# isl-org/adaptive-surface-reconstruction

Measured on AMD Instinct MI355X. Metric: input points/sec to signed implicit values, higher is better.
Workload: dtype f32 via bf16x3 (24-bit operands, f32 accumulate)

## Files before the change

### adaptive-surface-reconstruction_amd/csrc/asr_api.hip

```cpp
#include <cmath>
#include <cstdlib>
#include <cstring>

#include <algorithm>
#include <functional>
#include <future>
#include <mutex>
#include <thread>

#include "asr_common.h"
#include "asr_uset.h"

#define ASR_ROW_GROUP_SEGMENT (ctx->opt.row_segment > 0 ? ctx->opt.row_segment : (i64)524288)
#define CTX_GUARD(ctx)                                                  \
    if (!(ctx)) return ASR_HIP_EINVAL;                                  \
    (ctx)->err.clear();                                                 \
    if (hipSetDevice((ctx)->device) != hipSuccess) {                    \
        (ctx)->err = "hipSetDevice failed for the context's device";   \
        return ASR_HIP_EHIP;                                            \
    }

namespace {
struct OptEntry {
    const char* name;
    const char* env;
    i64 AsrOptions::*field;
};
const OptEntry k_options[] = {
        {"sconv_min_blocks", "ASR_SCONV_MIN_BLOCKS", &AsrOptions::sconv_min_blocks},
        {"sconv_wide_min", "ASR_SCONV_WIDE_MIN", &AsrOptions::sconv_wide_min},
        {"row_segment", "ASR_ROW_SEGMENT", &AsrOptions::row_segment},
        {"row_lpt", "ASR_ROW_LPT", &AsrOptions::row_lpt},
        {"row_ranked", "ASR_ROW_RANKED", &AsrOptions::row_ranked},
        {"sconv_plan", "ASR_SCONV_PLAN", &AsrOptions::sconv_plan},
        {"plan_arena", "ASR_PLAN_ARENA", &AsrOptions::plan_arena},
        {"sconv16_min_blocks", "ASR_SCONV16_MIN_BLOCKS", &AsrOptions::sconv16_min_blocks},
        {"knn_cells", "ASR_KNN_CELLS", &AsrOptions::knn_cells},
        {"knn_deep", "ASR_KNN_DEEP", &AsrOptions::knn_deep},
        {"search_hash_level", "ASR_SEARCH_HASH_LEVEL", &AsrOptions::search_hash_level},
        {"overlap", "ASR_OVERLAP", &AsrOptions::overlap},
        {"build_search", "ASR_BUILD_SEARCH", &AsrOptions::build_search},
        {"cconv_valu", "ASR_CCONV_VALU", &AsrOptions::cconv_valu},
        {"search_half", "ASR_SEARCH_HALF", &AsrOptions::search_half},
        {"search_priority", "ASR_SEARCH_PRIORITY", &AsrOptions::search_priority},
        {"shard_timing", "ASR_SHARD_TIMING", &AsrOptions::shard_timing},
        {"shard_geometry", "ASR_SHARD_GEOMETRY", &AsrOptions::shard_geometry},
        {"early_sort", "ASR_EARLY_SORT", &AsrOptions::early_sort},
        {"early_cells", "ASR_EARLY_CELLS", &AsrOptions::early_cells},
        {"sconv_split_rows", "ASR_SCONV_SPLIT_ROWS", &AsrOptions::sconv_split_rows},
        {"sconv_split_min_rows", "ASR_SCONV_SPLIT_MIN_ROWS", &AsrOptions::sconv_split_min_rows},
        {"arena_cap_mb", "ASR_ARENA_CAP_MB", &AsrOptions::arena_cap_mb},
        {"inject_failure", "ASR_INJECT_FAILURE", &AsrOptions::inject_failure},
};
void apply_arena_cap(asr_hip_context* ctx) {
    const size_t cap = ctx->opt.arena_cap_mb > 0 ? (size_t)ctx->opt.arena_cap_mb << 20 : 0;
    for (asr_hip_context* c : {ctx, ctx->aux})
        if (c) c->persist.cap = c->scratch.cap = c->shard_mem.cap = cap;
}

struct PrintSlot {
    asr_hip_print_callback cb = nullptr;
    void* user = nullptr;
};
std::mutex g_print_mu;
PrintSlot g_print[4];
}

extern "C" {

const char* asr_hip_version(void) { return "0.2.0+mi355x.r6"; }

int asr_hip_set_print_callback(asr_hip_print_callback callback, void* user, const int* levels, int num_levels) {
    if (num_levels < 0 || (num_levels > 0 && !levels)) return ASR_HIP_EINVAL;
    for (int i = 0; i < num_levels; ++i)
        if (levels[i] < ASR_HIP_DEBUG || levels[i] > ASR_HIP_ERROR) return ASR_HIP_EINVAL;
    std::lock_guard<std::mutex> lock(g_print_mu);
    for (int i = 0; i < num_levels; ++i) g_print[levels[i]] = PrintSlot{callback, callback ? user : nullptr};
    return ASR_HIP_OK;
}
void asr_hip_print(const char* msg, int level) {
    if (!msg || level < ASR_HIP_DEBUG || level > ASR_HIP_ERROR) return;
    PrintSlot s;
    {
        std::lock_guard<std::mutex> lock(g_print_mu);
        s = g_print[level];
    }
    if (s.cb) s.cb(msg, s.user);
}

size_t asr_hip_struct_size(const char* name) {
    if (!name) return 0;
    if (!strcmp(name, "asr_octree_frame")) return sizeof(asr_octree_frame);
    if (!strcmp(name, "asr_sparse_conv_args")) return sizeof(asr_sparse_conv_args);
    if (!strcmp(name, "asr_weight")) return sizeof(asr_weight);
    if (!strcmp(name, "asr_implicit_params")) return sizeof(asr_implicit_params);
    if (!strcmp(name, "asr_implicit_sizes")) return sizeof(asr_implicit_sizes);
    if (!strcmp(name, "asr_shard_comm")) return sizeof(asr_shard_comm);
    if (!strcmp(name, "asr_shard_stats")) return sizeof(asr_shard_stats);
    if (!strcmp(name, "asr_mesh_topology")) return sizeof(asr_mesh_topology);
    return 0;
}

int asr_hip_context_create(asr_hip_context** out, void* stream) {
    if (!out) return ASR_HIP_EINVAL;
    *out = nullptr;
    int ndev = 0;
    if (hipGetDeviceCount(&ndev) != hipSuccess || ndev <= 0) return ASR_HIP_ENODEV;
    asr_hip_context* ctx = new asr_hip_context();
    ctx->stream = (hipStream_t)stream;
    (void)hipGetDevice(&ctx->device);
    memset(&ctx->sizes, 0, sizeof(ctx->sizes));
    for (const OptEntry& o : k_options)
        if (const char* e = getenv(o.env)) ctx->opt.*(o.field) = atoll(e);
    apply_arena_cap(ctx);
    *out = ctx;
    return ASR_HIP_OK;
// ... 1661 lines not shown
```

### adaptive-surface-reconstruction_amd/csrc/asr_common.h

```cpp
#pragma once
#include <hip/hip_runtime.h>

#include <cstdint>
#include <cstdio>
#include <map>
#include <string>
#include <tuple>
#include <vector>

#include "../../include/asr_hip.h"

typedef uint64_t u64;
typedef int64_t i64;
typedef uint32_t u32;

struct Arena {
    struct Slab {
        char* base;
        size_t size, used;
    };
    std::vector<Slab> slabs;
    size_t min_slab = size_t(256) << 20;
    size_t cap = 0;

    void* alloc(size_t bytes) {
        bytes = (bytes + 255) & ~size_t(255);
        if (bytes == 0) bytes = 256;
        for (auto& s : slabs)
            if (s.size - s.used >= bytes) {
                void* p = s.base + s.used;
                s.used += bytes;
                return p;
            }
        size_t sz = bytes > min_slab ? bytes : min_slab;
        if (cap && reserved() + sz > cap) return nullptr;
        void* p = nullptr;
        if (hipMalloc(&p, sz) != hipSuccess) return nullptr;
        slabs.push_back({(char*)p, sz, bytes});
        return p;
    }
    void reset() {
        for (auto& s : slabs) s.used = 0;
    }
    size_t reserved() const {
        size_t t = 0;
        for (auto& s : slabs) t += s.size;
        return t;
    }
    void release() {
        for (auto& s : slabs) (void)hipFree(s.base);
        slabs.clear();
    }
};

struct ArenaMark {
    std::vector<size_t> used;
};
static inline void arena_mark(const Arena& a, ArenaMark& m) {
    m.used.clear();
    for (auto& s : a.slabs) m.used.push_back(s.used);
}
static inline void arena_rewind(Arena& a, const ArenaMark& m) {
    for (size_t i = 0; i < a.slabs.size(); ++i) a.slabs[i].used = i < m.used.size() ? m.used[i] : 0;
}

struct GridDev {
    i64 v = 0, p = 0;
    u64* keys = nullptr;
    float* centers = nullptr;
    float* sizes = nullptr;
    int32_t* nidx = nullptr;
    uint8_t* nkidx = nullptr;
    i64* nrs = nullptr;
    int32_t* up_idx = nullptr;
    uint8_t* up_kidx = nullptr;
    i64* up_rs = nullptr;
    int32_t* down_idx = nullptr;
    uint8_t* down_kidx = nullptr;
    i64* down_rs = nullptr;
    int32_t* perm_nb = nullptr;
    int32_t* perm_up = nullptr;
    int32_t* perm_down = nullptr;
};

struct AsrOptions {
    i64 sconv_min_blocks = 2816;
    i64 sconv16_min_blocks = 1024;
    i64 sconv_wide_min = 2048;
    i64 row_segment = 524288;
    i64 search_hash_level = -1;
    i64 knn_deep = 1;
    i64 knn_cells = 1;
    i64 plan_arena = 0;
    i64 sconv_plan = 1;
    i64 row_ranked = 1;
    i64 row_lpt = 1;
    i64 overlap = 1;
    i64 cconv_valu = 0;
    i64 build_search = 1;
    i64 shard_geometry = -1;
    i64 shard_timing = 0;
    i64 search_priority = 2;
    i64 search_half = 1;
    i64 early_cells = 1;
    i64 early_sort = 1;
    i64 arena_cap_mb = 0;
    i64 inject_failure = 0;
    i64 sconv_split_min_rows = 2048;
    i64 sconv_split_rows = 32768;
};

struct asr_conv_plan_view {
    const uint4* hdr;
    const int32_t* pool;
    i64 groups;
    unsigned pool_bytes;
};
struct asr_conv_plan {
    uint4* hdr = nullptr;
    int32_t* pool = nullptr;
    i64 groups = 0, groups_pad = 0, blocks = 0;
    i64* offs = nullptr;
    const int32_t* nidx = nullptr;
    const uint8_t* kidx = nullptr;
    const i64* rs = nullptr;
    const int32_t* perm = nullptr;
    i64 num_out = 0;
    int K = 0;
    bool usable() const { return hdr && blocks * 64 < (i64(1) << 32) - 65536; }
    asr_conv_plan_view view() const { return {hdr, pool, groups, (unsigned)(blocks * 64)}; }
};

struct AsrPointIndex {
    bool valid = false;
    const float* pts = nullptr;
    const float* radii = nullptr;
    i64 n = 0;
    int lsort = 0;
    float4* sorted = nullptr;
    int32_t* ids = nullptr;
    int32_t* rank = nullptr;
    float* srad = nullptr;
    u64* codes = nullptr;
    u64* tab_keys = nullptr;
    u64 tab_mask = 0;
    int32_t* tab_start = nullptr;
    int32_t* tab_end = nullptr;
    int tab_lmin = 0, tab_lmax = -1, tab_lhash = 0, tab_grow = 0;
};

struct asr_hip_context {
    hipStream_t stream = nullptr;
    std::string err;
    AsrOptions opt;
    std::map<const void*, asr_conv_plan> conv_plans;
    std::map<std::string, i64> sconv_launches;
    ArenaMark build_mark;
    bool build_mark_ok = false;
    Arena persist;
    Arena scratch;
    Arena plan_arena;
    uint64_t plan_arena_epoch = 0;
    u64* nodes = nullptr;
    u64* leaves = nullptr;
    i64 num_nodes = 0, num_leaves = 0;
    asr_octree_frame frame;
    asr_implicit_sizes sizes;
    GridDev grids[ASR_NUM_GRIDS];
    int32_t* agg_idx = nullptr;
    float* agg_dist = nullptr;
    float* agg_compat = nullptr;
    i64* agg_rs = nullptr;
    int32_t* agg_spos = nullptr;
    const float4* agg_sorted = nullptr;
    bool has_search = false;
    bool build_sharded = false;
    const int32_t* agg_rows = nullptr;
    i64 agg_nq = 0;
    const float* agg_qcenters = nullptr;
// ... 306 lines not shown
```

### adaptive-surface-reconstruction_amd/csrc/asr_geom.hip

```cpp
#include <cstdlib>
#include <cstring>
#include <algorithm>
#include <rocprim/rocprim.hpp>

#include "asr_common.h"
#include "asr_prim.h"

namespace {
using namespace asr_prim;

constexpr int BLK = 256;

struct HashTab {
    u64* keys;
    int32_t* vals;
    u64 mask;
};

struct TabProbe {
    u64 bucket, step, low, bmask;
    __device__ inline u64 slot() const { return ((bucket & bmask) << 6) | low; }
    __device__ inline void next() { bucket += step; }
};
__device__ inline TabProbe tab_probe(const HashTab& t, u64 key) {
    const u64 h = asr_hash64(key >> 6);
    return TabProbe{h, (h >> 32) | 1, key & 63, t.mask >> 6};
}

__device__ inline u64 ld_agent(const u64* p) {
    return __hip_atomic_load(p, __ATOMIC_RELAXED, __HIP_MEMORY_SCOPE_AGENT);
}

__device__ inline int tab_insert(const HashTab& t, u64 key, u64* slot_out = nullptr) {
    TabProbe pr = tab_probe(t, key);
    for (u64 probe = 0; probe <= pr.bmask; ++probe, pr.next()) {
        const u64 slot = pr.slot();
        u64 cur = ld_agent(&t.keys[slot]);
        if (cur == 0) {
            cur = atomicCAS((unsigned long long*)&t.keys[slot], 0ull, (unsigned long long)key);
            if (cur == 0) {
                if (slot_out) *slot_out = slot;
                return 1;
            }
        }
        if (cur == key) {
            if (slot_out) *slot_out = slot;
            return 0;
        }
    }
    return -1;
}
__device__ inline int tab_insert_shared(const HashTab& t, u64 key) {
    TabProbe pr = tab_probe(t, key);
    for (u64 probe = 0; probe <= pr.bmask; ++probe, pr.next()) {
        const u64 slot = pr.slot();
        u64 cur = t.keys[slot];
        if (cur == 0) cur = ld_agent(&t.keys[slot]);
        if (cur == 0) {
            cur = atomicCAS((unsigned long long*)&t.keys[slot], 0ull, (unsigned long long)key);
            if (cur == 0) return 1;
        }
        if (cur == key) return 0;
    }
    return -1;
}
__device__ inline bool tab_contains(const HashTab& t, u64 key) {
    TabProbe pr = tab_probe(t, key);
    for (u64 probe = 0; probe <= pr.bmask; ++probe, pr.next()) {
        const u64 slot = pr.slot();
        const u64 cur = t.keys[slot];
        if (cur == key) return true;
        if (cur == 0) return false;
    }
    return false;
}
__device__ inline int tab_find(const HashTab& t, u64 key) {
    TabProbe pr = tab_probe(t, key);
    for (u64 probe = 0; probe <= pr.bmask; ++probe, pr.next()) {
        const u64 slot = pr.slot();
        const u64 cur = t.keys[slot];
        if (cur == key) return t.vals[slot];
        if (cur == 0) return -1;
    }
    return -1;
}
__device__ inline i64 tab_find_slot(const HashTab& t, u64 key) {
    TabProbe pr = tab_probe(t, key);
    for (u64 probe = 0; probe <= pr.bmask; ++probe, pr.next()) {
        const u64 slot = pr.slot();
// ... 1770 lines not shown
    const int j = rg_job_of(b, c * 128);
    const i64 r0 = c * 128 - b.base[j];
    u64 m0 = masks[sorted_ids[c * 128 + lane]], m1 = masks[sorted_ids[c * 128 + 64 + lane]];
#pragma unroll
    for (int o = 32; o > 0; o >>= 1) {
        m0 |= __shfl_xor(m0, o, 64);
        m1 |= __shfl_xor(m1, o, 64);
    }
    if (lane == 0) {
        int cost = __popcll(m0) + __popcll(m1);
        if (r0 + 128 > b.v[j]) cost = 0;
        ckey[c] = (int32_t)(((i64)j << 13) | ((r0 / seg) << 7) | (127 - cost));
        cid[c] = (int32_t)c;
    }
}
__global__ void k_rg_apply(RowGroupBatch b, const int32_t* sorted_ids, const int32_t* order, int lpt) {
    const i64 e = blockIdx.x * (i64)blockDim.x + threadIdx.x;
    if (e >= b.base[b.n]) return;
    const int j = rg_job_of(b, e);
    const i64 r = e - b.base[j];
    if (r >= b.v[j]) return;
    const i64 src = lpt ? (i64)order[e >> 7] * 128 + (e & 127) : e;
    b.out[j][r] = (int32_t)(sorted_ids[src] - b.base[j]);
}

constexpr int RG_MAX_MASKS = 16384;
constexpr int RG_MASK_TAB = 65536;
__global__ void k_rg_masks(RowGroupBatch b, u64* masks, HashTab t, int* cnt) {
    const i64 e = blockIdx.x * (i64)blockDim.x + threadIdx.x;
    if (e >= b.base[b.n]) return;
    const int j = rg_job_of(b, e);
    const i64 r = e - b.base[j];
    u64 m = 0;
    if (r < b.v[j]) {
        const i64* rs = b.rs[j];
        const uint8_t* kidx = b.kidx[j];
        for (i64 p = rs[r]; p < rs[r + 1]; ++p) m |= u64(1) << (kidx[p] & 63);
        if (tab_insert_shared(t, (m >> 1) + 1) < 0) cnt[1] = 1;
    }
    masks[e] = m;
}
__global__ void k_rg_mask_collect(HashTab t, u64* list, int32_t* slot_of, int* cnt) {
    const u64 i = blockIdx.x * (u64)blockDim.x + threadIdx.x;
    const u64 k = i <= t.mask ? t.keys[i] : 0;
    const int o = block_append(k != 0, cnt + 2);
    if (k && o < RG_MAX_MASKS) {
        list[o] = k;
        slot_of[o] = (int32_t)i;
    }
}
__global__ __launch_bounds__(256) void k_rg_mask_ranks(HashTab t, const u64* list, const int32_t* slot_of, const int* cnt) {
    __shared__ u64 s_key[2048];
    const int n = cnt[2];
    if (n > RG_MAX_MASKS) return;
    const int i = blockIdx.x * blockDim.x + threadIdx.x;
    if (blockIdx.x * blockDim.x >= n) return;
    const u64 mine = i < n ? list[i] : 0;
    int rank = 0;
    for (int base = 0; base < n; base += 2048) {
        __syncthreads();
        for (int e = threadIdx.x; e < 2048; e += blockDim.x) s_key[e] = base + e < n ? list[base + e] : ~u64(0);
        __syncthreads();
        const int m = min(2048, n - base);
        for (int e = 0; e < m; ++e) rank += s_key[e] < mine;
    }
    if (i < n) t.vals[slot_of[i]] = rank;
}
__global__ void k_rg_keys_ranked(RowGroupBatch b, i64 seg, const u64* masks, HashTab t, unsigned* keys, int32_t* ids,
                                 int rank_bits) {
    const i64 e = blockIdx.x * (i64)blockDim.x + threadIdx.x;
    if (e >= b.base[b.n]) return;
    const int j = rg_job_of(b, e);
    const i64 r = e - b.base[j];
    unsigned key;
    if (r < b.v[j]) {
        const int rank = tab_find(t, (masks[e] >> 1) + 1);
        key = ((unsigned)j << (6 + rank_bits)) | ((unsigned)(r / seg) << rank_bits) | (unsigned)rank;
    } else {
        key = ((unsigned)j << (6 + rank_bits)) | (63u << rank_bits) | ((1u << rank_bits) - 1u);
    }
    keys[e] = key;
    ids[e] = (int32_t)e;
}

__device__ inline u64 dev_morton_add(u64 a, u64 b) {
    const u64 M = 0x9249249249249249ull;
    u64 c = ((a | ~M) + (b & M)) & M;
    c |= ((a | ~(M << 1)) + (b & (M << 1))) & (M << 1);
    c |= ((a | ~(M << 2)) + (b & (M << 2))) & (M << 2);
    return c;
}
__device__ inline u64 dev_morton_sub(u64 a, u64 b) {
    const u64 M = 0x9249249249249249ull;
    u64 c = ((a & M) - (b & M)) & M;
    c |= ((a & (M << 1)) - (b & (M << 1))) & (M << 1);
    c |= ((a & (M << 2)) - (b & (M << 2))) & (M << 2);
    return c;
}
__device__ inline int node_lookup(const HashTab& t, u64 key) {
    TabProbe pr = tab_probe(t, key);
    for (u64 probe = 0; probe <= pr.bmask; ++probe, pr.next()) {
        const u64 slot = pr.slot();
        const u64 cur = t.keys[slot];
        if (cur == key) return t.vals[slot];
        if (cur == 0) return -2;
    }
    return -2;
}
__device__ inline bool dual_owned(const HashTab& t, u64 key, int i, u64& vertex_key) {
    const u64 IM = 0x9249249249249249ull;
    const int lev = asr_key_level(key);
    const u64 min_lev_key = u64(1) << (3 * lev);
    const u64 vk = dev_morton_add(key, (u64)i);
    const u64 vk_ = vk - min_lev_key;
    if (vk >= (min_lev_key << 1) || !(vk_ & IM) || !(vk_ & (IM << 1)) || !(vk_ & (IM << 2))) return false;
    vertex_key = vk;
    for (int j = 0; j < 8; ++j) {
        if (j == i) continue;
        const u64 ak = dev_morton_sub(vk, (u64)j);
        const int r = node_lookup(t, ak);
        if (r == -2) continue;
        if (r == -1) return false;
        if (ak < key) return false;
    }
    return true;
}
__global__ void k_dual_count(const u64* leaves, i64 v, HashTab t, i64* counts) {
    i64 q = blockIdx.x * (i64)blockDim.x + threadIdx.x;
    if (q > v) return;
    if (q == v) {
        counts[v] = 0;
        return;
    }
    const u64 key = leaves[q];
    int n = 0;
    u64 vk;
    for (int i = 0; i < 8; ++i) n += dual_owned(t, key, i, vk) ? 1 : 0;
    counts[q] = n;
}
__global__ void k_dual_fill(const u64* leaves, i64 v, HashTab t, const i64* offsets, i64* out, int* cnt) {
    i64 q = blockIdx.x * (i64)blockDim.x + threadIdx.x;
    if (q >= v) return;
    const u64 key = leaves[q];
    i64 o = offsets[q];
    for (int i = 0; i < 8; ++i) {
        u64 vk;
        if (!dual_owned(t, key, i, vk)) continue;
        for (int j = 0; j < 8; ++j) {
            u64 k = dev_morton_sub(vk, (u64)j);
            int r = -2;
            while (k != 0 && (r = node_lookup(t, k)) == -2) k >>= 3;
            if (k == 0 || r < 0) {
                cnt[1] = 1;
                r = -1;
            }
            out[o * 8 + j] = r;
        }
        ++o;
    }
}

int make_table(asr_hip_context* ctx, Arena& arena, u64 cap, bool with_vals, HashTab& t) {
    t.keys = arena_alloc<u64>(arena, cap);
    t.vals = with_vals ? arena_alloc<int32_t>(arena, cap) : nullptr;
    t.mask = cap - 1;
    if (!t.keys || (with_vals && !t.vals)) ASR_FAIL(ctx, ASR_HIP_EHIP, "arena allocation failed");
// ... 364 lines not shown
        ASR_CHECK_LAUNCH(ctx);
        k_chunk_key<<<grid_for(nc, BLK), BLK, 0, ctx->stream>>>(tcost, v, seg, ckey, cid);
        ASR_CHECK_LAUNCH(ctx);
        ASR_TRY((sort_pairs<int32_t, int32_t>(ctx, ctx->scratch, ckey, ckey_s, cid, cid_s, nc,
                                              7 + bits_for((v + seg - 1) / seg + 1))));
        k_chunk_apply<<<grid_for(v, BLK), BLK, 0, ctx->stream>>>(perm_m, cid_s, v, perm_out);
        ASR_CHECK_LAUNCH(ctx);
    }
    return ASR_HIP_OK;
}

static int rg_batch_run(asr_hip_context* ctx, const asr_row_group_job* jobs, int n, i64 seg, int mask_bits);
static int rg_batch_run_ranked(asr_hip_context* ctx, const asr_row_group_job* jobs, int n, i64 seg, bool* done);
int asr_geom_row_groups_batch(asr_hip_context* ctx, const asr_row_group_job* jobs, int n, i64 seg) {
    if (seg < 128) seg = 128;
    bool fits = n <= RG_MAX_JOBS && seg % 128 == 0;
    for (int j = 0; j < n && fits; ++j) fits = jobs[j].v / seg < 63 && jobs[j].v < (i64(1) << 31);
    if (!fits) {
        for (int j = 0; j < n; ++j)
            ASR_TRY(asr_geom_row_groups(ctx, jobs[j].kidx, jobs[j].rs, jobs[j].v, seg, jobs[j].perm_out, jobs[j].kbits));
        return ASR_HIP_OK;
    }
    if (ctx->opt.row_ranked) {
        bool done = false;
        ASR_TRY(rg_batch_run_ranked(ctx, jobs, n, seg, &done));
        if (done) return ASR_HIP_OK;
    }
    std::vector<asr_row_group_job> small_jobs, wide_jobs;
    for (int j = 0; j < n; ++j) (jobs[j].kbits <= 10 ? small_jobs : wide_jobs).push_back(jobs[j]);
    if (!small_jobs.empty()) ASR_TRY(rg_batch_run(ctx, small_jobs.data(), (int)small_jobs.size(), seg, 9));
    if (!wide_jobs.empty()) ASR_TRY(rg_batch_run(ctx, wide_jobs.data(), (int)wide_jobs.size(), seg, 54));
    return ASR_HIP_OK;
}
static int rg_batch_run_ranked(asr_hip_context* ctx, const asr_row_group_job* jobs, int n, i64 seg, bool* done) {
    *done = false;
    ASR_TRY(ensure_flags(ctx));
    RowGroupBatch b;
    b.n = 0;
    i64 total = 0;
    for (int j = 0; j < n; ++j) {
        if (jobs[j].v <= 0) continue;
        b.base[b.n] = total;
        b.v[b.n] = jobs[j].v;
        b.kidx[b.n] = jobs[j].kidx;
        b.rs[b.n] = jobs[j].rs;
        b.out[b.n] = jobs[j].perm_out;
        total += (jobs[j].v + 127) / 128 * 128;
        ++b.n;
    }
    if (b.n == 0) {
        *done = true;
        return ASR_HIP_OK;
    }
    b.base[b.n] = total;
    if (total >= (i64(1) << 31)) ASR_FAIL(ctx, ASR_HIP_EINVAL, "row_groups: too many rows");
    u64* masks = arena_alloc<u64>(ctx->scratch, total);
    unsigned* keys = arena_alloc<unsigned>(ctx->scratch, total);
    unsigned* keys_s = arena_alloc<unsigned>(ctx->scratch, total);
    int32_t* ids = arena_alloc<int32_t>(ctx->scratch, total);
    int32_t* ids_s = arena_alloc<int32_t>(ctx->scratch, total);
    const i64 nc = total / 128;
    int32_t* ckey = arena_alloc<int32_t>(ctx->scratch, nc);
    int32_t* ckey_s = arena_alloc<int32_t>(ctx->scratch, nc);
    int32_t* cid = arena_alloc<int32_t>(ctx->scratch, nc);
    int32_t* cid_s = arena_alloc<int32_t>(ctx->scratch, nc);
    if (!masks || !keys || !keys_s || !ids || !ids_s || !ckey || !ckey_s || !cid || !cid_s)
        ASR_FAIL(ctx, ASR_HIP_EHIP, "arena allocation failed");
    HashTab t;
    ASR_TRY(make_table(ctx, ctx->scratch, RG_MASK_TAB, true, t));
    ASR_TRY(fresh_flags(ctx));
    k_rg_masks<<<grid_for(total, BLK), BLK, 0, ctx->stream>>>(b, masks, t, ctx->d_flags);
    ASR_CHECK_LAUNCH(ctx);
    u64* mlist = arena_alloc<u64>(ctx->scratch, RG_MAX_MASKS);
    int32_t* mslot = arena_alloc<int32_t>(ctx->scratch, RG_MAX_MASKS);
    if (!mlist || !mslot) ASR_FAIL(ctx, ASR_HIP_EHIP, "arena allocation failed");
    k_rg_mask_collect<<<grid_for((i64)t.mask + 1, BLK), BLK, 0, ctx->stream>>>(t, mlist, mslot, ctx->d_flags);
    ASR_CHECK_LAUNCH(ctx);
    k_rg_mask_ranks<<<RG_MAX_MASKS / 256, 256, 0, ctx->stream>>>(t, mlist, mslot, ctx->d_flags);
    ASR_CHECK_LAUNCH(ctx);
    int host[16];
    ASR_TRY(read_flags(ctx, host));
    if (host[1] || host[2] > RG_MAX_MASKS) return ASR_HIP_OK;
    const int rank_bits = bits_for(std::max(host[2], 2));
    k_rg_keys_ranked<<<grid_for(total, BLK), BLK, 0, ctx->stream>>>(b, seg, masks, t, keys, ids, rank_bits);
    ASR_CHECK_LAUNCH(ctx);
    ASR_TRY((sort_pairs<unsigned, int32_t>(ctx, ctx->scratch, keys, keys_s, ids, ids_s, total, 4 + 6 + rank_bits)));
    const int lpt = ctx->opt.row_lpt != 0;
    if (lpt) {
        k_rg_chunk_keys<<<grid_for(nc * 64, BLK), BLK, 0, ctx->stream>>>(b, seg, ids_s, masks, ckey, cid);
        ASR_CHECK_LAUNCH(ctx);
        ASR_TRY((sort_pairs<int32_t, int32_t>(ctx, ctx->scratch, ckey, ckey_s, cid, cid_s, nc, 17)));
    }
    k_rg_apply<<<grid_for(total, BLK), BLK, 0, ctx->stream>>>(b, ids_s, cid_s, lpt);
    ASR_CHECK_LAUNCH(ctx);
    *done = true;
    return ASR_HIP_OK;
}
static int rg_batch_run(asr_hip_context* ctx, const asr_row_group_job* jobs, int n, i64 seg, int mask_bits) {
    RowGroupBatch b;
    b.n = 0;
    i64 total = 0;
    for (int j = 0; j < n; ++j) {
        if (jobs[j].v <= 0) continue;
        b.base[b.n] = total;
        b.v[b.n] = jobs[j].v;
        b.kidx[b.n] = jobs[j].kidx;
        b.rs[b.n] = jobs[j].rs;
        b.out[b.n] = jobs[j].perm_out;
        total += (jobs[j].v + 127) / 128 * 128;
        ++b.n;
    }
    if (b.n == 0) return ASR_HIP_OK;
    b.base[b.n] = total;
    if (total >= (i64(1) << 31)) ASR_FAIL(ctx, ASR_HIP_EINVAL, "row_groups: too many rows");
    u64* keys = arena_alloc<u64>(ctx->scratch, total);
    u64* keys_s = arena_alloc<u64>(ctx->scratch, total);
    u64* masks = arena_alloc<u64>(ctx->scratch, total);
    int32_t* ids = arena_alloc<int32_t>(ctx->scratch, total);
    int32_t* ids_s = arena_alloc<int32_t>(ctx->scratch, total);
    const i64 nc = total / 128;
    int32_t* ckey = arena_alloc<int32_t>(ctx->scratch, nc);
    int32_t* ckey_s = arena_alloc<int32_t>(ctx->scratch, nc);
    int32_t* cid = arena_alloc<int32_t>(ctx->scratch, nc);
    int32_t* cid_s = arena_alloc<int32_t>(ctx->scratch, nc);
    if (!keys || !keys_s || !masks || !ids || !ids_s || !ckey || !ckey_s || !cid || !cid_s)
        ASR_FAIL(ctx, ASR_HIP_EHIP, "arena allocation failed");
    k_rg_keys<<<grid_for(total, BLK), BLK, 0, ctx->stream>>>(b, seg, keys, masks, ids, mask_bits);
    ASR_CHECK_LAUNCH(ctx);
    ASR_TRY((sort_pairs<u64, int32_t>(ctx, ctx->scratch, keys, keys_s, ids, ids_s, total, 4 + 6 + mask_bits)));
    const int lpt = ctx->opt.row_lpt != 0;
    if (lpt) {
        k_rg_chunk_keys<<<grid_for(nc * 64, BLK), BLK, 0, ctx->stream>>>(b, seg, ids_s, masks, ckey, cid);
        ASR_CHECK_LAUNCH(ctx);
        ASR_TRY((sort_pairs<int32_t, int32_t>(ctx, ctx->scratch, ckey, ckey_s, cid, cid_s, nc, 17)));
    }
    k_rg_apply<<<grid_for(total, BLK), BLK, 0, ctx->stream>>>(b, ids_s, cid_s, lpt);
    ASR_CHECK_LAUNCH(ctx);
    return ASR_HIP_OK;
}

static int coarsen_scan(asr_hip_context* ctx, const u64* keys, i64 v, u64** pre, i64* v_out) {
    u64* packed = arena_alloc<u64>(ctx->scratch, v + 1);
    *pre = arena_alloc<u64>(ctx->scratch, v + 2);
    if (!packed || !*pre) ASR_FAIL(ctx, ASR_HIP_EHIP, "arena allocation failed");
    k_coarsen_flags<<<grid_for(v + 1, BLK), BLK, 0, ctx->stream>>>(keys, v, packed);
    ASR_CHECK_LAUNCH(ctx);
    size_t tb = 0;
    ASR_HIP_CHECK(ctx, rocprim::exclusive_scan(nullptr, tb, packed, *pre, u64(0), (size_t)(v + 1), rocprim::plus<u64>(),
                                               ctx->stream));
    void* tmp = ctx->scratch.alloc(tb ? tb : 256);
    if (!tmp) ASR_FAIL(ctx, ASR_HIP_EHIP, "arena allocation failed");
    ASR_HIP_CHECK(ctx, rocprim::exclusive_scan(tmp, tb, packed, *pre, u64(0), (size_t)(v + 1), rocprim::plus<u64>(),
                                               ctx->stream));
    u64 totals = 0;
    ASR_HIP_CHECK(ctx, hipMemcpyAsync(&totals, *pre + v, sizeof(u64), hipMemcpyDeviceToHost, ctx->stream));
    ASR_HIP_CHECK(ctx, hipStreamSynchronize(ctx->stream));
    *v_out = (i64)(totals & 0xffffffffu) + (i64)(totals >> 32);
    return ASR_HIP_OK;
}
static int coarsen_lists(asr_hip_context* ctx, const u64* keys, i64 v, const u64* pre, i64 vo, int32_t* src,
                         u64* out_keys, int32_t* up_idx, uint8_t* up_kidx, i64* up_rs, int32_t* down_idx,
                         uint8_t* down_kidx, i64* down_rs) {
    k_coarsen_place<<<grid_for(v, BLK), BLK, 0, ctx->stream>>>(keys, v, pre, out_keys, src);
    ASR_CHECK_LAUNCH(ctx);
    k_coarsen_up<<<grid_for(vo, BLK), BLK, 0, ctx->stream>>>(keys, v, src, vo, up_idx, up_kidx);
    ASR_CHECK_LAUNCH(ctx);
    k_iota64<<<grid_for(v + 1, BLK), BLK, 0, ctx->stream>>>(up_rs, v + 1);
    ASR_CHECK_LAUNCH(ctx);
    if (!down_rs) return ASR_HIP_OK;
    i64* cnt = arena_alloc<i64>(ctx->scratch, vo + 1);
    if (!cnt) ASR_FAIL(ctx, ASR_HIP_EHIP, "arena allocation failed");
    k_coarsen_down_count<<<grid_for(vo + 1, BLK), BLK, 0, ctx->stream>>>(keys, v, src, vo, cnt);
    ASR_CHECK_LAUNCH(ctx);
    ASR_TRY(scan_counts(ctx, ctx->scratch, cnt, down_rs, vo + 1));
// ... 951 lines not shown
```

Measured before the change: 275.4 million.

## Replace global radix sort of row-group keys with segmented stable radix sort

Adds a custom segmented LSD radix sort (count, per-segment offset scan, stable scatter using wave ballots) over 7-bit digits. It replaces the full-width rocprim sort_pairs on composite job/segment/rank keys for both the row permutation and the LPT chunk ordering. Because segments are already contiguous, only the rank bits need sorting, which cuts sort passes and key width. It adds custom kernels, risks correctness when there are more than 16 jobs, and uses one or two passes depending on rank_bits.

New measurement: 275.8 million (median of 3 runs). Within noise of the previous version (+0.1%).

```diff
diff --git a/adaptive-surface-reconstruction_amd/csrc/asr_api.hip b/adaptive-surface-reconstruction_amd/csrc/asr_api.hip
--- a/adaptive-surface-reconstruction_amd/csrc/asr_api.hip
+++ b/adaptive-surface-reconstruction_amd/csrc/asr_api.hip
@@ -32,6 +32,7 @@
         {"row_segment", "ASR_ROW_SEGMENT", &AsrOptions::row_segment},
         {"row_lpt", "ASR_ROW_LPT", &AsrOptions::row_lpt},
         {"row_ranked", "ASR_ROW_RANKED", &AsrOptions::row_ranked},
+        {"row_sort", "ASR_ROW_SORT", &AsrOptions::row_sort},
         {"sconv_plan", "ASR_SCONV_PLAN", &AsrOptions::sconv_plan},
         {"plan_arena", "ASR_PLAN_ARENA", &AsrOptions::plan_arena},
         {"sconv16_min_blocks", "ASR_SCONV16_MIN_BLOCKS", &AsrOptions::sconv16_min_blocks},
diff --git a/adaptive-surface-reconstruction_amd/csrc/asr_common.h b/adaptive-surface-reconstruction_amd/csrc/asr_common.h
--- a/adaptive-surface-reconstruction_amd/csrc/asr_common.h
+++ b/adaptive-surface-reconstruction_amd/csrc/asr_common.h
@@ -95,6 +95,7 @@
     i64 sconv_plan = 1;
     i64 row_ranked = 1;
     i64 row_lpt = 1;
+    i64 row_sort = 1;
     i64 overlap = 1;
     i64 cconv_valu = 0;
     i64 build_search = 1;
diff --git a/adaptive-surface-reconstruction_amd/csrc/asr_geom.hip b/adaptive-surface-reconstruction_amd/csrc/asr_geom.hip
--- a/adaptive-surface-reconstruction_amd/csrc/asr_geom.hip
+++ b/adaptive-surface-reconstruction_amd/csrc/asr_geom.hip
@@ -5,6 +5,7 @@
 
 #include "asr_common.h"
 #include "asr_prim.h"
+#include "asr_segsort.h"
 
 namespace {
 using namespace asr_prim;
@@ -1941,6 +1942,12 @@
     keys[e] = key;
     ids[e] = (int32_t)e;
 }
+__global__ void k_rg_ranks(RowGroupBatch b, const u64* masks, HashTab t, unsigned* ranks) {
+    const i64 e = blockIdx.x * (i64)blockDim.x + threadIdx.x;
+    if (e >= b.base[b.n]) return;
+    const int j = rg_job_of(b, e);
+    ranks[e] = e - b.base[j] < b.v[j] ? (unsigned)tab_find(t, (masks[e] >> 1) + 1) : 0u;
+}
 
 __device__ inline u64 dev_morton_add(u64 a, u64 b) {
     const u64 M = 0x9249249249249249ull;
@@ -2471,14 +2478,40 @@
     ASR_TRY(read_flags(ctx, host));
     if (host[1] || host[2] > RG_MAX_MASKS) return ASR_HIP_OK;
     const int rank_bits = bits_for(std::max(host[2], 2));
-    k_rg_keys_ranked<<<grid_for(total, BLK), BLK, 0, ctx->stream>>>(b, seg, masks, t, keys, ids, rank_bits);
-    ASR_CHECK_LAUNCH(ctx);
-    ASR_TRY((sort_pairs<unsigned, int32_t>(ctx, ctx->scratch, keys, keys_s, ids, ids_s, total, 4 + 6 + rank_bits)));
     const int lpt = ctx->opt.row_lpt != 0;
-    if (lpt) {
-        k_rg_chunk_keys<<<grid_for(nc * 64, BLK), BLK, 0, ctx->stream>>>(b, seg, ids_s, masks, ckey, cid);
+    if (ctx->opt.row_sort) {
+        asr_segsort::Plan rows, chunks;
+        asr_segsort::plan_init(rows, seg);
+        asr_segsort::plan_init(chunks, seg / 128);
+        for (int j = 0; j < b.n; ++j) {
+            asr_segsort::plan_add(rows, b.base[j], b.v[j], b.base[j + 1]);
+            asr_segsort::plan_add(chunks, b.base[j] / 128, (b.base[j + 1] - b.base[j]) / 128, b.base[j + 1] / 128);
+        }
+        int* row_tab = arena_alloc<int>(ctx->scratch, asr_segsort::table_ints(rows));
+        int* chunk_tab = arena_alloc<int>(ctx->scratch, asr_segsort::table_ints(chunks));
+        if (!row_tab || !chunk_tab) ASR_FAIL(ctx, ASR_HIP_EHIP, "arena allocation failed");
+        k_rg_ranks<<<grid_for(total, BLK), BLK, 0, ctx->stream>>>(b, masks, t, keys);
         ASR_CHECK_LAUNCH(ctx);
-        ASR_TRY((sort_pairs<int32_t, int32_t>(ctx, ctx->scratch, ckey, ckey_s, cid, cid_s, nc, 17)));
+        if (rank_bits <= 7) {
+            ASR_TRY(asr_segsort::pass(ctx, rows, keys, 0, nullptr, ids_s, row_tab));
+        } else {
+            ASR_TRY(asr_segsort::pass(ctx, rows, keys, 0, nullptr, ids, row_tab));
+            ASR_TRY(asr_segsort::pass(ctx, rows, keys, 7, ids, ids_s, row_tab));
+        }
+        if (lpt) {
+            k_rg_chunk_keys<<<grid_for(nc * 64, BLK), BLK, 0, ctx->stream>>>(b, seg, ids_s, masks, ckey, cid);
+            ASR_CHECK_LAUNCH(ctx);
+            ASR_TRY(asr_segsort::pass(ctx, chunks, (const unsigned*)ckey, 0, nullptr, cid_s, chunk_tab));
+        }
+    } else {
+        k_rg_keys_ranked<<<grid_for(total, BLK), BLK, 0, ctx->stream>>>(b, seg, masks, t, keys, ids, rank_bits);
+        ASR_CHECK_LAUNCH(ctx);
+        ASR_TRY((sort_pairs<unsigned, int32_t>(ctx, ctx->scratch, keys, keys_s, ids, ids_s, total, 4 + 6 + rank_bits)));
+        if (lpt) {
+            k_rg_chunk_keys<<<grid_for(nc * 64, BLK), BLK, 0, ctx->stream>>>(b, seg, ids_s, masks, ckey, cid);
+            ASR_CHECK_LAUNCH(ctx);
+            ASR_TRY((sort_pairs<int32_t, int32_t>(ctx, ctx->scratch, ckey, ckey_s, cid, cid_s, nc, 17)));
+        }
     }
     k_rg_apply<<<grid_for(total, BLK), BLK, 0, ctx->stream>>>(b, ids_s, cid_s, lpt);
     ASR_CHECK_LAUNCH(ctx);
diff --git a/adaptive-surface-reconstruction_amd/csrc/asr_segsort.h b/adaptive-surface-reconstruction_amd/csrc/asr_segsort.h
--- /dev/null
+++ b/adaptive-surface-reconstruction_amd/csrc/asr_segsort.h
@@ -0,0 +1,191 @@
+#pragma once
+#include "asr_common.h"
+
+namespace asr_segsort {
+
+constexpr int MAX_JOBS = 16, CHUNK = 2048, BINS = 128, WAVES = 4, SLICES = 8;
+constexpr int STEPS = CHUNK / WAVES / 64;
+constexpr int BATCH = 32;
+
+struct Plan {
+    int n;
+    int chunks_per_seg;
+    i64 seg_len;
+    i64 base[MAX_JOBS];
+    i64 count[MAX_JOBS];
+    i64 end[MAX_JOBS];
+    int chunk_base[MAX_JOBS + 1];
+    int seg_base[MAX_JOBS + 1];
+};
+static inline bool plan_add(Plan& p, i64 base, i64 count, i64 end) {
+    if (count <= 0) return true;
+    if (p.n >= MAX_JOBS || p.seg_len <= 0) return false;
+    const int j = p.n++;
+    p.base[j] = base;
+    p.count[j] = count;
+    p.end[j] = end;
+    const i64 whole = count / p.seg_len, rest = count - whole * p.seg_len;
+    p.chunk_base[j + 1] = p.chunk_base[j] + (int)(whole * p.chunks_per_seg + (rest + CHUNK - 1) / CHUNK);
+    p.seg_base[j + 1] = p.seg_base[j] + (int)(whole + (rest > 0));
+    return true;
+}
+static inline void plan_init(Plan& p, i64 seg_len) {
+    p.n = 0;
+    p.seg_len = seg_len;
+    p.chunks_per_seg = (int)((seg_len + CHUNK - 1) / CHUNK);
+    p.chunk_base[0] = p.seg_base[0] = 0;
+}
+static inline size_t table_ints(const Plan& p) { return (size_t)p.chunk_base[p.n] * (WAVES + 1) * BINS; }
+
+namespace {
+__device__ inline int chunk_range(const Plan& p, int c, i64& lo, i64& hi) {
+    int j = 0;
+    while (j + 1 < p.n && c >= p.chunk_base[j + 1]) ++j;
+    const int lc = c - p.chunk_base[j];
+    const i64 s = lc / p.chunks_per_seg, k = lc % p.chunks_per_seg;
+    const i64 seg_hi = min((s + 1) * p.seg_len, p.count[j]);
+    lo = p.base[j] + s * p.seg_len + k * CHUNK;
+    hi = min(lo + CHUNK, p.base[j] + seg_hi);
+    return j;
+}
+__device__ inline u64 same_digit(unsigned d, bool ok) {
+    u64 peers = __ballot(ok);
+#pragma unroll
+    for (int b = 0; b < 7; ++b) {
+        const u64 set = __ballot((d >> b) & 1u);
+        peers &= ((d >> b) & 1u) ? set : ~set;
+    }
+    return peers;
+}
+__device__ inline void wave_step_fence() {
+    __builtin_amdgcn_fence(__ATOMIC_ACQ_REL, "wavefront");
+    __builtin_amdgcn_wave_barrier();
+}
+
+__global__ __launch_bounds__(256) void k_segsort_count(Plan p, const unsigned* key, int shift, const int32_t* in,
+                                                       int* table) {
+    __shared__ int s_cnt[WAVES][BINS];
+    const int c = blockIdx.x, w = threadIdx.x >> 6, lane = threadIdx.x & 63;
+    i64 lo, hi;
+    chunk_range(p, c, lo, hi);
+    s_cnt[w][lane] = 0;
+    s_cnt[w][lane + 64] = 0;
+    __syncthreads();
+    const u64 below = (u64(1) << lane) - 1;
+    const i64 wlo = lo + (i64)w * (CHUNK / WAVES);
+    for (int s = 0; s < STEPS && wlo + s * 64 < hi; ++s) {
+        const i64 e = wlo + s * 64 + lane;
+        const bool ok = e < hi;
+        const unsigned d = ok ? (key[in ? in[e] : (int32_t)e] >> shift) & 127u : 0u;
+        const u64 peers = same_digit(d, ok);
+        if (ok && !(peers & below)) atomicAdd(&s_cnt[w][d], __popcll(peers));
+    }
+    __syncthreads();
+    int* row = table + ((size_t)c * WAVES + w) * BINS;
+    row[lane] = s_cnt[w][lane];
+    row[lane + 64] = s_cnt[w][lane + 64];
+    if (threadIdx.x < BINS) {
+        int sum = 0;
+#pragma unroll
+        for (int q = 0; q < WAVES; ++q) sum += s_cnt[q][threadIdx.x];
+        table[((size_t)gridDim.x * WAVES + c) * BINS + threadIdx.x] = sum;
+    }
+}
+
+__global__ __launch_bounds__(SLICES * BINS) void k_segsort_offsets(Plan p, int chunks, int* table) {
+    __shared__ int s_part[SLICES][BINS];
+    __shared__ int s_low[SLICES];
+    const int g = threadIdx.x >> 7, d = threadIdx.x & 127, lane = threadIdx.x & 63;
+    int j = 0;
+    while (j + 1 < p.n && (int)blockIdx.x >= p.seg_base[j + 1]) ++j;
+    const i64 s = (int)blockIdx.x - p.seg_base[j];
+    const i64 seg_lo = s * p.seg_len, seg_hi = min(seg_lo + p.seg_len, p.count[j]);
+    const int rows = (int)((seg_hi - seg_lo + CHUNK - 1) / CHUNK);
+    int* t = table + ((size_t)chunks * WAVES + (size_t)p.chunk_base[j] + (size_t)s * p.chunks_per_seg) * BINS + d;
+    const int per = (rows + SLICES - 1) / SLICES;
+    const int r_lo = min(g * per, rows), r_hi = min(r_lo + per, rows);
+    int x[BATCH];
+    int sum = 0;
+    for (int r0 = r_lo; r0 < r_hi; r0 += BATCH) {
+#pragma unroll
+        for (int k = 0; k < BATCH; ++k) x[k] = r0 + k < r_hi ? t[(size_t)(r0 + k) * BINS] : 0;
+#pragma unroll
+        for (int k = 0; k < BATCH; ++k) sum += x[k];
+    }
+    s_part[g][d] = sum;
+    __syncthreads();
+    int before = 0, total = 0;
+#pragma unroll
+    for (int q = 0; q < SLICES; ++q) {
+        const int y = s_part[q][d];
+        before += q < g ? y : 0;
+        total += y;
+    }
+    int incl = total;
+#pragma unroll
+    for (int o = 1; o < 64; o <<= 1) {
+        const int up = __shfl_up(incl, o, 64);
+        if (lane >= o) incl += up;
+    }
+    if (d == 63) s_low[g] = incl;
+    __syncthreads();
+    int run = (int)(p.base[j] + seg_lo) + incl - total + (d >= 64 ? s_low[g] : 0) + before;
+    for (int r0 = r_lo; r0 < r_hi; r0 += BATCH) {
+        if (r_hi - r_lo > BATCH) {
+#pragma unroll
+            for (int k = 0; k < BATCH; ++k) x[k] = r0 + k < r_hi ? t[(size_t)(r0 + k) * BINS] : 0;
+        }
+#pragma unroll
+        for (int k = 0; k < BATCH; ++k) {
+            if (r0 + k < r_hi) t[(size_t)(r0 + k) * BINS] = run;
+            run += x[k];
+        }
+    }
+}
+
+__global__ __launch_bounds__(256) void k_segsort_scatter(Plan p, const unsigned* key, int shift, const int32_t* in,
+                                                         const int* table, int32_t* out) {
+    __shared__ int s_pos[WAVES][BINS];
+    const int c = blockIdx.x, w = threadIdx.x >> 6, lane = threadIdx.x & 63;
+    i64 lo, hi;
+    const int j = chunk_range(p, c, lo, hi);
+#pragma unroll
+    for (int h = 0; h < BINS; h += 64) {
+        int pos = table[((size_t)gridDim.x * WAVES + c) * BINS + h + lane];
+        for (int q = 0; q < w; ++q) pos += table[((size_t)c * WAVES + q) * BINS + h + lane];
+        s_pos[w][h + lane] = pos;
+    }
+    __syncthreads();
+    const u64 below = (u64(1) << lane) - 1;
+    const i64 wlo = lo + (i64)w * (CHUNK / WAVES);
+    for (int s = 0; s < STEPS && wlo + s * 64 < hi; ++s) {
+        const i64 e = wlo + s * 64 + lane;
+        const bool ok = e < hi;
+        const int32_t v = ok ? (in ? in[e] : (int32_t)e) : 0;
+        const unsigned d = ok ? (key[v] >> shift) & 127u : 0u;
+        const u64 peers = same_digit(d, ok);
+        if (ok) out[s_pos[w][d] + __popcll(peers & below)] = v;
+        wave_step_fence();
+        if (ok && !(peers >> lane >> 1)) s_pos[w][d] += __popcll(peers);
+        wave_step_fence();
+    }
+    if (hi == p.base[j] + p.count[j])
+        for (i64 e = hi + threadIdx.x; e < p.end[j]; e += blockDim.x) out[e] = in ? in[e] : (int32_t)e;
+}
+
+}
+
+static inline int pass(asr_hip_context* ctx, const Plan& p, const unsigned* key, int shift, const int32_t* in,
+                       int32_t* out, int* table) {
+    if (p.n == 0) return ASR_HIP_OK;
+    const int chunks = p.chunk_base[p.n], segs = p.seg_base[p.n];
+    k_segsort_count<<<chunks, 256, 0, ctx->stream>>>(p, key, shift, in, table);
+    ASR_CHECK_LAUNCH(ctx);
+    k_segsort_offsets<<<segs, SLICES * BINS, 0, ctx->stream>>>(p, chunks, table);
+    ASR_CHECK_LAUNCH(ctx);
+    k_segsort_scatter<<<chunks, 256, 0, ctx->stream>>>(p, key, shift, in, table, out);
+    ASR_CHECK_LAUNCH(ctx);
+    return ASR_HIP_OK;
+}
+
+}
```
